# redmod-team/SympGPR

Measured on AMD Instinct MI355X. Metric: Gram-build GB/s + Cholesky fp64 TFLOP/s at N=65536 d=2; |alpha-alpha_ref|/|alpha_ref|, higher is better.
Workload: dtype f64

## Files before the change

include/sympgpr_probe.h:

```cpp
#ifndef SYMPGPR_PROBE_H
#define SYMPGPR_PROBE_H
#include <stddef.h>
#ifdef __cplusplus
extern "C" {
#endif

int sgpr_probe_mfma_f64(int waves_per_simd, int iters, double *tflops);
int sgpr_probe_hbm_write(size_t bytes, int reps, double *gbs);
int sgpr_probe_mfma_clock(int nacc, int waves_per_simd, int iters, double *out3);
int sgpr_probe_gemm(int m, int n, int k, int lower, double *out4);
int sgpr_probe_gemm_debug(int bits);
int sgpr_probe_leaf(double *out8);
int sgpr_probe_lat(double *out8);
int sgpr_probe_xcc(int nblocks, int *host_out);
int sgpr_probe_cumask(const unsigned *mask_words, int nwords, int nblocks, int *host_out);

int sgpr_probe_generated_eval(int family, int which, int m, const double *xa, const double *ya,
                              const double *xb, const double *yb, const double *l, int nl, double *out);

int sgpr_probe_queue_plan(int n, int nworkers, int *starts_out, int max_starts, unsigned *tasks_out, int max_tasks,
                          int *counts);
int sgpr_probe_queue_plan_partial(int n, int nworkers, int nq, int *starts_out, int max_starts, unsigned *tasks_out,
                                  int max_tasks, int *counts);
int sgpr_probe_queue_trace_begin(int max_tasks);
int sgpr_probe_queue_trace_end(unsigned long long *out, int max_tasks);
int sgpr_probe_queue_trace_clear(void);
int sgpr_probe_queue_postmortem(int always);
int sgpr_probe_queue_force_giveup(int on);
int sgpr_probe_tune(const char *name, double value);
int sgpr_probe_strassen_plan(int m, int n, int k, int lower, long smin, long kslab, long scratch_doubles, long long *out,
                             int max_records, int *count);
int sgpr_probe_gemm_strassen_dev(int m, int n, int k, double alpha, const double *A, size_t lda, const double *B, size_t ldb,
                                 double beta, double *C, size_t ldc, int lower, void *stream);
int sgpr_probe_gemm_nt2_dev(int m, int n, int k, double alpha, const double *A, size_t lda, const double *B, size_t ldb,
                            double beta, double *C, size_t ldc, double alpha2, double *C2, size_t ldc2, void *stream);
int sgpr_probe_strassen2_plan(int m, int n, int k, int lower, long smin, long kslab, long smin2, long kslab2, long scratch_doubles,
                              long long *out, int max_records, int *count);
int sgpr_probe_gemm_nt4_dev(int m, int n, int k, const double *A, size_t lda, const double *B, size_t ldb, double beta, int count,
                            double *const *C, const size_t *ldc, const double *alpha, void *stream);
int sgpr_probe_strassen_rec_plan(int m, int n, int k, int lower, long scratch_doubles, long cfg_out[5], long long *out,
                                 int max_records, int *count);
int sgpr_probe_strassen_rec_scratch(int n, unsigned long long out[2]);
int sgpr_probe_gemm_strassen_rec_dev(int m, int n, int k, double alpha, const double *A, size_t lda, const double *B, size_t ldb,
                                     double beta, double *C, size_t ldc, int lower, void *stream);
int sgpr_probe_batch_layout(int path, int mode, int d, int reg, int nbatch, int n_pts, int nhyp, unsigned long long out[24]);
unsigned sgpr_probe_map_calls(void);
int sgpr_probe_map_team(int ntest, int n0);

int sgpr_probe_trsm_piece(int ticket, int cap, int strips, int out[5]);
int sgpr_probe_trsm_counts(int strips, int cap, unsigned long long out[2]);

int sgpr_probe_census(int na, int threads_a, int lds_a, int spin_a, const unsigned *mask_a, int nwords_a,
                      int nb, int threads_b, int lds_b, int spin_b, const unsigned *mask_b, int nwords_b,
                      unsigned long long *host_out);

#ifdef __cplusplus
}
#endif
#endif
```

sympgpr_amd/_lib.py:

```python
import ctypes as C
import os

import numpy as np

FAMILIES = {"A": 0, "B": 1, "C": 2, "D": 3, "USER": 4}
K_KERN, K_DXDX0, K_DYDY0, K_DXDY0 = 0, 1, 2, 3
K_DLX, K_DLY = 4, 8
K_DX, K_DY, K_DX0, K_DY0, K_DXDX0DY0, K_DYDY0DY0, K_DXDY0DY0 = 16, 17, 18, 19, 20, 21, 22
G_QQ, G_PQ, G_QP, G_PP, G_ALL, G_LOWER, G_OCML, G_DLX, G_DLY = 1, 2, 4, 8, 15, 16, 32, 64, 128
FIT_LOWER_ONLY, FIT_REG, FIT_BLOCK_QQ, FIT_BLOCK_PP = 1, 4, 8, 16
MAP_WRAP_Q, MAP_WRAP_P, MAP_EXPLICIT, MAP_LOSS_NEGP = 1, 2, 4, 8
E_ARG, E_NODEVICE, E_HIP, E_NOMEM, E_STATE = -1, -2, -3, -4, -5
LOO_LPD, LOO_PRESS = 0, 1

ABI_VERSION = 5
_dp = C.POINTER(C.c_double)
_vp = C.c_void_p


class SympGPRError(RuntimeError):
    code = None
    detail = ""


# ... 135 lines not shown
    "sgpr_probe_queue_plan_partial": (C.c_int, [C.c_int, C.c_int, C.c_int, C.POINTER(C.c_int), C.c_int, C.POINTER(C.c_uint),
                                                C.c_int, C.POINTER(C.c_int)]),
    "sgpr_probe_queue_trace_begin": (C.c_int, [C.c_int]),
    "sgpr_probe_queue_trace_end": (C.c_int, [C.POINTER(C.c_ulonglong), C.c_int]),
    "sgpr_probe_queue_postmortem": (C.c_int, [C.c_int]),
    "sgpr_probe_queue_force_giveup": (C.c_int, [C.c_int]),
    "sgpr_probe_tune": (C.c_int, [C.c_char_p, C.c_double]),
    "sgpr_probe_map_calls": (C.c_uint, []),
    "sgpr_probe_map_team": (C.c_int, [C.c_int, C.c_int]),
    "sgpr_probe_trsm_piece": (C.c_int, [C.c_int, C.c_int, C.c_int, C.POINTER(C.c_int)]),
    "sgpr_probe_trsm_counts": (C.c_int, [C.c_int, C.c_int, C.POINTER(C.c_ulonglong)]),
    "sgpr_probe_queue_trace_clear": (C.c_int, []),
    "sgpr_probe_strassen_plan": (C.c_int, [C.c_int, C.c_int, C.c_int, C.c_int, C.c_long, C.c_long, C.c_long,
                                           C.POINTER(C.c_longlong), C.c_int, C.POINTER(C.c_int)]),
    "sgpr_probe_gemm_strassen_dev": (C.c_int, [C.c_int, C.c_int, C.c_int, C.c_double, C.c_void_p, C.c_size_t, C.c_void_p, C.c_size_t,
                                               C.c_double, C.c_void_p, C.c_size_t, C.c_int, C.c_void_p]),
    "sgpr_probe_gemm_nt2_dev": (C.c_int, [C.c_int, C.c_int, C.c_int, C.c_double, C.c_void_p, C.c_size_t, C.c_void_p, C.c_size_t,
                                          C.c_double, C.c_void_p, C.c_size_t, C.c_double, C.c_void_p, C.c_size_t, C.c_void_p]),
    "sgpr_probe_strassen2_plan": (C.c_int, [C.c_int, C.c_int, C.c_int, C.c_int, C.c_long, C.c_long, C.c_long, C.c_long, C.c_long,
                                            C.POINTER(C.c_longlong), C.c_int, C.POINTER(C.c_int)]),
    "sgpr_probe_strassen_rec_plan": (C.c_int, [C.c_int, C.c_int, C.c_int, C.c_int, C.c_long, C.POINTER(C.c_long),
                                               C.POINTER(C.c_longlong), C.c_int, C.POINTER(C.c_int)]),
    "sgpr_probe_strassen_rec_scratch": (C.c_int, [C.c_int, C.POINTER(C.c_ulonglong)]),
    "sgpr_probe_gemm_strassen_rec_dev": (C.c_int, [C.c_int, C.c_int, C.c_int, C.c_double, C.c_void_p, C.c_size_t, C.c_void_p, C.c_size_t,
                                                   C.c_double, C.c_void_p, C.c_size_t, C.c_int, C.c_void_p]),
    "sgpr_probe_gemm_nt4_dev": (C.c_int, [C.c_int, C.c_int, C.c_int, C.c_void_p, C.c_size_t, C.c_void_p, C.c_size_t, C.c_double, C.c_int,
                                          C.POINTER(C.c_void_p), C.POINTER(C.c_size_t), C.POINTER(C.c_double), C.c_void_p]),
    "sgpr_probe_batch_layout": (C.c_int, [C.c_int, C.c_int, C.c_int, C.c_int, C.c_int, C.c_int, C.c_int,
                                          C.POINTER(C.c_ulonglong)]),
    "sgpr_probe_census": (C.c_int, [C.c_int, C.c_int, C.c_int, C.c_int, C.POINTER(C.c_uint), C.c_int,
                                    C.c_int, C.c_int, C.c_int, C.c_int, C.POINTER(C.c_uint), C.c_int,
                                    C.POINTER(C.c_ulonglong)]),
}

_LIB = None
_PROBE = None


def load_library():
    global _LIB
    if _LIB is not None:
        return _LIB
    path = lib_path()
    if os.environ.get("SYMPGPR_NO_TORCH_PRELOAD") != "1":
        try:
            import torch
# ... 80 lines not shown
```

sympgpr_amd/csrc/chol.hip:

```cpp
#include <algorithm>
#include <cstdlib>
#include <mutex>
#include <vector>

#include "cholq.h"
#include "common.h"
#include "gemm_tile.h"
#include "leaf.h"

namespace sgpr {

namespace {

using namespace leaf;


__global__ __launch_bounds__(LT) void leaf_kernel(int nb, double *A, size_t lda, double *inv,
                                                  int *dinfo, int goff, int mode,
                                                  unsigned long long *stamps)
{
    __shared__ double s[LEAF_LDS];
    if (nb == LEAF) leaf_body(s, (int)LEAF, A, lda, inv, dinfo, goff, mode, stamps);
    else            leaf_body(s, nb, A, lda, inv, dinfo, goff, mode, stamps);
}
// ... 958 lines not shown
    int dev = -1;
    if (caller) {
        SGPR_HIP(hipStreamGetDevice(caller, &dev));
    } else {
        SGPR_HIP(hipGetDevice(&dev));
    }
    if (dev < 0 || dev >= 64) { set_error("potrf: device index out of range"); return SGPR_E_ARG; }
    std::lock_guard<std::mutex> lock(g_side_mu);
    if (!side[dev]) {
        int cur = -1, lo = 0, hi = 0;
        SGPR_HIP(hipGetDevice(&cur));
        if (cur != dev) SGPR_HIP(hipSetDevice(dev));
        hipError_t e = hipDeviceGetStreamPriorityRange(&lo, &hi);
        if (e == hipSuccess) e = hipStreamCreateWithPriority(&side[dev], hipStreamNonBlocking, hi);
        if (e == hipSuccess) register_exit_release();
        if (cur != dev) (void)hipSetDevice(cur);
        SGPR_HIP(e);
    }
    *out = side[dev];
    *dev_out = dev;
    return 0;
}

struct QueueDevice {
    std::mutex mu;
    hipEvent_t done = nullptr;
    int ncu = 0;
    hipStream_t workers[4] = {}, panels[4] = {};
    bool overlap_ok[4] = {};
    bool failed = false;
};
QueueDevice g_qdev[64];

__global__ void overlap_probe_kernel(int *w, int me)
{
    __hip_atomic_store((gint *)(w + me), 1, __ATOMIC_RELAXED, __HIP_MEMORY_SCOPE_AGENT);
    const unsigned long long t0 = __builtin_amdgcn_s_memrealtime();
    int seen = 0;
    while (!(seen = __hip_atomic_load((gint *)(w + 1 - me), __ATOMIC_RELAXED, __HIP_MEMORY_SCOPE_AGENT))) {
        __builtin_amdgcn_s_sleep(32);
        if (__builtin_amdgcn_s_memrealtime() - t0 > 5000000ull) break;
    }
    w[2 + me] = seen ? 1 : 2;
}
static bool queue_overlap_ok(hipStream_t sw, hipStream_t sp)
{
// ... 117 lines not shown
    cholq::remember(ws, n, (int)(plan->tasks.size() / 2));
    cholq::remember_plan(plan);
    static const bool qdebug = tune("q_debug", 0) != 0;
    if (qdebug) {
        SGPR_HIP(hipStreamSynchronize(su));
        cholq::postmortem(false);
    }
    if (plan->nq < plan->nblk) {
        const int S = plan->starts[plan->nq];
        Ctx ct = c;
        ct.qws = nullptr;
        static const bool nosync = tune("q_nosync", 0) != 0;
        if (!nosync) SGPR_HIP(hipStreamSynchronize(su));
        return potrf_lookahead(n - S, A + S + (size_t)S * lda, lda, ct, 0, off0 + S);
    }
    return 0;
}

void release_all_streams_at_exit()
{
    int ndev = 0;
    if (hipGetDeviceCount(&ndev) != hipSuccess) { (void)hipGetLastError(); return; }
    for (int dev = 0; dev < ndev && dev < 64; ++dev) {
        hipStream_t drop[9] = {};
        int nd = 0;
        {
            std::lock_guard<std::mutex> lock(g_side_mu);
            if (g_side[dev]) { drop[nd++] = g_side[dev]; g_side[dev] = nullptr; }
        }
        {
            QueueDevice &qd = g_qdev[dev];
            std::lock_guard<std::mutex> lock(qd.mu);
            for (int r = 0; r < 4; ++r) {
                if (qd.workers[r]) { drop[nd++] = qd.workers[r]; qd.workers[r] = nullptr; }
                if (qd.panels[r]) { drop[nd++] = qd.panels[r]; qd.panels[r] = nullptr; }
            }
            qd.failed = true;
        }
        if (!nd) continue;
        int cur = -1;
        (void)hipGetDevice(&cur);
        if (cur != dev) (void)hipSetDevice(dev);
        for (int q = 0; q < nd; ++q) (void)hipStreamDestroy(drop[q]);
        if (cur != dev && cur >= 0) (void)hipSetDevice(cur);
    }
    (void)hipGetLastError();
}

int release_streams(int dev)
{
    {
        bool any = false;
        {
            std::lock_guard<std::mutex> lock(g_side_mu);
            any = g_side[dev] != nullptr;
        }
        QueueDevice &qd = g_qdev[dev];
        std::lock_guard<std::mutex> lock(qd.mu);
        for (int r = 0; r < 4; ++r) any = any || qd.workers[r] || qd.panels[r];
        any = any || qd.done;
        if (!any) return 0;
    }
    int cur = -1;
    SGPR_HIP(hipGetDevice(&cur));
    if (cur != dev) SGPR_HIP(hipSetDevice(dev));
    hipError_t first = hipSuccess;
    auto drop = [&](hipStream_t &s) {
        if (!s) return;
        hipError_t e = hipStreamSynchronize(s);
        if (e == hipSuccess) e = hipStreamDestroy(s);
        if (e != hipSuccess && first == hipSuccess) first = e;
        s = nullptr;
    };
    {
        std::lock_guard<std::mutex> lock(g_side_mu);
        drop(g_side[dev]);
    }
    {
        QueueDevice &qd = g_qdev[dev];
        std::lock_guard<std::mutex> lock(qd.mu);
        for (int r = 0; r < 4; ++r) { drop(qd.workers[r]); drop(qd.panels[r]); }
        if (qd.done) {
            const hipError_t e = hipEventDestroy(qd.done);
            if (e != hipSuccess && first == hipSuccess) first = e;
            qd.done = nullptr;
        }
        qd.ncu = 0;
        qd.failed = false;
        for (int r = 0; r < 4; ++r) qd.overlap_ok[r] = false;
    }
    if (cur != dev) (void)hipSetDevice(cur);
    SGPR_HIP(first);
    return 0;
}

int potrf_lookahead(int n, double *A, size_t lda, const Ctx &c, int nb, int off0)
{
    if (nb == 0 && c.qws && c.flags && cholq::eligible(n) && (lda & 1) == 0 && (((uintptr_t)A & 15) == 0) && off0 % LEAF == 0) {
        const int rq = potrf_queue(n, A, lda, c, off0);
// ... 446 lines not shown
```

sympgpr_amd/csrc/common.h:

```cpp
#pragma once
#include <hip/hip_runtime.h>
#include <cstddef>
#include <cstdint>
#include <string>
#include <type_traits>
#include <vector>

#include "../../include/sympgpr_hip.h"

namespace sgpr {

void set_error(const std::string &msg);
double tune(const char *name, double dflt);
void tune_set(const char *name, double v);
int hip_fail(hipError_t e, const char *what, const char *file, int line);

#define SGPR_HIP(call)                                                          \
    do {                                                                        \
        hipError_t e__ = (call);                                                \
        if (e__ != hipSuccess) return ::sgpr::hip_fail(e__, #call, __FILE__, __LINE__); \
    } while (0)

#define SGPR_CHECK_LAUNCH() SGPR_HIP(hipGetLastError())

// ... 84 lines not shown
int gemm_nt_two(int m, int n, int k, double alpha, const double *A, size_t lda, const double *B, size_t ldb, double beta,
             double *C, size_t ldc, double alpha2, double *C2, size_t ldc2, hipStream_t st);
constexpr int STRASSEN_REC = 16;
enum { PLAN_SUM = 1, PLAN_PROD = 2, PLAN_CLASSIC = 3 };
int gemm_nt_strassen(int m, int n, int k, double alpha, const double *A, size_t lda, const double *B, size_t ldb, double beta,
                     double *C, size_t ldc, int lower, hipStream_t st);
int strassen_plan(int m, int n, int k, int lower, long smin, long kslab, size_t scratch_doubles, std::vector<long long> &out);
enum { PLAN2_SUM = 4, PLAN2_PROD = 5 };
int strassen_outer_plan(int m, int n, int k, int lower, long smin, long kslab, long smin2, long kslab2, size_t scratch_doubles,
                   std::vector<long long> &out);
int gemm_nt_multi(int m, int n, int k, const double *A, size_t lda, const double *B, size_t ldb, double beta, int count,
                  double *const *C, const size_t *ldc, const double *alpha, hipStream_t st);
size_t strassen_scratch_doubles(int m, int n, int k, int lower, int levels);
struct StrassenCfg { long smin = -1, kslab = -1, smin2 = -1, kslab2 = -1, smin_under = -1; };
int gemm_nt_strassen_cfg(int m, int n, int k, double alpha, const double *A, size_t lda, const double *B, size_t ldb, double beta,
                         double *C, size_t ldc, int lower, const StrassenCfg &cfg, hipStream_t st);
size_t strassen_scratch_doubles_cfg(int m, int n, int k, int lower, int levels, const StrassenCfg &cfg);
struct StrassenRec { bool on = false; long smin_gemm = 0, smin_syrk = 0, smin2_gemm = 0, smin2_syrk = 0, kslab = 0, kslab2 = 0, kslab2_short = 0; };
StrassenRec strassen_rec_values();
StrassenCfg strassen_rec_cfg(const StrassenRec &v, int k, int lower);
int strassen_rec_plan(int m, int n, int k, int lower, long cfg_out[5], size_t scratch_doubles, std::vector<long long> &out);
int gemm_nt_strassen_rec(int m, int n, int k, double alpha, const double *A, size_t lda, const double *B, size_t ldb, double beta,
                         double *C, size_t ldc, int lower, hipStream_t st);
void potrf_strassen_need(int n, size_t out[2]);
void strassen_reserve(size_t both, size_t one, hipStream_t st);
int strassen_trim();
int gemm_profile_begin();
int gemm_profile_end(double *out12);
int gemm_profile_launches(double *buf, int max_records);
void gemm_set_overlap(int on);
int gemm_nt_diag(int m, int n, int k, double alpha, const double *A, size_t lda, const double *B, size_t ldb,
                 double beta, double *C, size_t ldc, int lower, unsigned long long *stamps, int dbg, hipStream_t st);

constexpr int LEAF = 128;
constexpr int POTRF_HANDOFF_TIMEOUT = -1000001;
constexpr int SOLVE_HANDOFF_TIMEOUT = -1000002;
inline int info_status(int info)
{
    if (info >= 0) return info;
    set_error(info == POTRF_HANDOFF_TIMEOUT ? "potrf: a hand-off inside the panel kernel timed out"
              : info == SOLVE_HANDOFF_TIMEOUT ? "solve: a hand-off between the strips of a triangular solve timed out" : "potrf: internal error");
    return SGPR_E_HIP;
}
size_t potrf_workspace(int n);
int potrf(int n, double *A, size_t lda, void *work, size_t lwork, int *dinfo, hipStream_t st);
size_t potrf_batch_flag_bytes(int nbatch);
// ... 123 lines not shown
```

sympgpr_amd/csrc/gemm_f64.hip:

```cpp
#include <algorithm>
#include <atomic>
#include <cstdlib>
#include <mutex>
#include <type_traits>
#include <vector>

#include "common.h"
#include "gemm_tile.h"

namespace sgpr {

namespace {

struct ProfRec { double flop; int big; int m, n, k, lower, overlap; };
struct Prof {
    std::mutex mu;
    std::atomic<bool> on{false};
    std::vector<hipEvent_t> pool;
    std::vector<ProfRec> recs;
    long dropped = 0;
};
constexpr int PROF_POOL = 8192;
Prof g_prof;
thread_local int t_overlap = 0;
// ... 495 lines not shown
    };
    PlanCfg ci = under_of(c);
    ci.scratch = ~(size_t)0;
    for (size_t i = 0; i + STRASSEN_REC <= plan.size(); i += STRASSEN_REC) {
        const long long *r = &plan[i];
        if (r[0] == PLAN_SUM) sums(r, 0);
        else if (r[0] == PLAN2_SUM) sums(r, 2);
        else if (r[0] == PLAN2_PROD) {
            inner_plan(r, ci, in);
            for (size_t j = 0; j + STRASSEN_REC <= in.size(); j += STRASSEN_REC)
                if (in[j] == PLAN_SUM) sums(&in[j], 0);
        }
    }
    return nd;
}

struct Scratch {
    std::mutex mu;
    double *p = nullptr;
    size_t cap = 0, failed = 0;
    hipEvent_t ev = nullptr;
    hipStream_t last = nullptr;
    bool used = false;
};
Scratch g_scratch[64];

bool scratch_ensure(Scratch &s, size_t need)
{
    static const bool forced_fail = tune("gemm_strassen_noscratch", 0) != 0;
    if (forced_fail) return false;
    if (s.cap >= need) return true;
    if (s.failed && need >= s.failed) return false;
    if (s.p) { (void)hipFree(s.p); s.p = nullptr; s.cap = 0; s.used = false; }
    if (hipMalloc((void **)&s.p, need * sizeof(double)) != hipSuccess) {
        (void)hipGetLastError();
        s.p = nullptr;
        s.failed = need;
        return false;
    }
    s.cap = need;
    return true;
}
int device_of(hipStream_t st)
{
    int dev = -1;
    if ((st ? hipStreamGetDevice(st, &dev) : hipGetDevice(&dev)) != hipSuccess) { (void)hipGetLastError(); return -1; }
    return (dev >= 0 && dev < 64) ? dev : -1;
}

int block_sum(int rows, int cols, const double *X, size_t ldx, const double *Y, size_t ldy, double sign, double *T, hipStream_t st)
{
    const long pieces = (long)((rows + 511) / 512) * ((cols + 3) / 4);
    hipLaunchKernelGGL(block_sum_kernel, dim3((unsigned)std::min(pieces, 2048L)), dim3(256), 0, st, rows, cols, X, ldx, Y, ldy, sign, T);
    SGPR_CHECK_LAUNCH();
    return 0;
}

int run_plan(const long long *recs, size_t nrec, double alpha, const double *A, size_t lda, const double *B, size_t ldb,
             double beta, double *C, size_t ldc, double alpha2, double *C2, size_t ldc2, double *SA, double *SB, hipStream_t st)
{
    for (size_t i = 0; i < nrec; ++i) {
        const long long *r = recs + i * STRASSEN_REC;
        int rc = 0;
        if (r[0] == PLAN_SUM) {
            const double *P = r[1] ? B : A;
            const size_t ld = r[1] ? ldb : lda;
            rc = block_sum((int)r[2], (int)r[3], P + r[4] + (size_t)r[5] * ld, ld, P + r[6] + (size_t)r[7] * ld, ld, (double)r[8],
                           r[1] ? SB : SA, st);
        } else if (r[0] == PLAN_PROD) {
            const int m = (int)r[7], n = (int)r[8], k = (int)r[9];
            const double *Ap = r[1] ? SA : A + r[2] + (size_t)r[3] * lda;
            const double *Bp = r[4] ? SB : B + r[5] + (size_t)r[6] * ldb;
            const size_t la = r[1] ? (size_t)m : lda, lb = r[4] ? (size_t)n : ldb;
            double *C1 = C + r[10] + (size_t)r[11] * ldc;
            if (C2) {
                double *cs[4] = {C1, nullptr, nullptr, nullptr};
                size_t ls[4] = {ldc, 0, 0, 0};
                double as[4] = {alpha * (double)r[12], 0.0, 0.0, 0.0};
                int cnt = 1;
                auto add = [&](double *p, size_t l, double a) { cs[cnt] = p; ls[cnt] = l; as[cnt] = a; ++cnt; };
                if (r[15]) add(C + r[13] + (size_t)r[14] * ldc, ldc, alpha * (double)r[15]);
                add(C2 + r[10] + (size_t)r[11] * ldc2, ldc2, alpha2 * (double)r[12]);
                if (r[15]) add(C2 + r[13] + (size_t)r[14] * ldc2, ldc2, alpha2 * (double)r[15]);
                if (cnt == 2) rc = gemm_nt_two(m, n, k, as[0], Ap, la, Bp, lb, 1.0, cs[0], ls[0], as[1], cs[1], ls[1], st);
                else          rc = gemm_nt_multi(m, n, k, Ap, la, Bp, lb, 1.0, cnt, cs, ls, as, st);
            } else if (r[15]) {
                rc = gemm_nt_two(m, n, k, alpha * (double)r[12], Ap, la, Bp, lb, 1.0, C1, ldc,
                                 alpha * (double)r[15], C + r[13] + (size_t)r[14] * ldc, ldc, st);
            } else {
                rc = gemm_nt(m, n, k, alpha * (double)r[12], Ap, la, Bp, lb, 1.0, C1, ldc, 0, 0, st);
            }
// ... 24 lines not shown
    std::vector<long long> in;
    for (size_t i = 0; i + STRASSEN_REC <= plan.size(); i += STRASSEN_REC) {
        const long long *r = &plan[i];
        int rc = 0;
        if (r[0] == PLAN2_SUM) {
            const double *P = r[1] ? B : A;
            const size_t ld = r[1] ? ldb : lda;
            rc = block_sum((int)r[2], (int)r[3], P + r[4] + (size_t)r[5] * ld, ld, P + r[6] + (size_t)r[7] * ld, ld, (double)r[8],
                           r[1] ? OB : OA, st);
        } else if (r[0] == PLAN2_PROD) {
            const double *X = r[1] ? OA : A + r[2] + (size_t)r[3] * lda;
            const double *Y = r[4] ? OB : B + r[5] + (size_t)r[6] * ldb;
            inner_plan(r, ci, in);
            rc = run_plan(in.data(), in.size() / STRASSEN_REC, alpha * (double)r[12], X, r[1] ? (size_t)r[7] : lda, Y, r[4] ? (size_t)r[8] : ldb,
                          1.0, C + r[10] + (size_t)r[11] * ldc, ldc, alpha * (double)r[15], r[15] ? C + r[13] + (size_t)r[14] * ldc : nullptr, ldc,
                          SA, SB, st);
        } else {
            rc = run_plan(r, 1, alpha, A, lda, B, ldb, beta, C, ldc, 0.0, nullptr, 0, SA, SB, st);
        }
        if (rc) return rc;
    }
    return 0;
}
}

int strassen_plan(int m, int n, int k, int lower, long smin, long kslab, size_t scratch_doubles, std::vector<long long> &out)
{
    if (m < 0 || n < 0 || k < 0 || (lower && m != n)) { set_error("strassen_plan: bad extents"); return SGPR_E_ARG; }
    PlanCfg c = default_cfg();
    if (smin >= 0) c.smin = std::max(128L, smin);
    if (kslab >= 0) c.kslab = std::max(32L, kslab);
    c.scratch = scratch_doubles;
    out.clear();
    if (lower) plan_syrk(n, k, 0, c, out);
    else       plan_gemm(m, n, k, 0, 0, 0, 0, c, out);
    return 0;
}

namespace {
Plan2Cfg cfg2_of(long smin, long kslab, long smin2, long kslab2, size_t scratch_doubles)
{
    Plan2Cfg c = default_cfg2();
    if (smin >= 0) c.in.smin = std::max(128L, smin);
    if (kslab >= 0) c.in.kslab = std::max(32L, kslab);
    if (smin2 >= 0) c.smin2 = std::max(256L, smin2);
    if (kslab2 >= 0) c.kslab2 = std::max(64L, kslab2);
// ... 37 lines not shown
    if (v.kslab2_short < 64 || v.kslab2_short % 64 != 0 || v.kslab2_short >= v.kslab2) v.kslab2_short = 0;
    return v;
}
StrassenCfg strassen_rec_cfg(const StrassenRec &v, int k, int lower)
{
    StrassenCfg c;
    if (!v.on) return c;
    c.smin = lower ? v.smin_syrk : v.smin_gemm;
    c.smin2 = lower ? v.smin2_syrk : v.smin2_gemm;
    c.smin_under = std::min(c.smin, c.smin2 / 2);
    c.kslab = v.kslab;
    c.kslab2 = (k < v.kslab2 && v.kslab2_short > 0 && k >= v.kslab2_short) ? v.kslab2_short : v.kslab2;
    return c;
}
int strassen_rec_plan(int m, int n, int k, int lower, long cfg_out[5], size_t scratch_doubles, std::vector<long long> &out)
{
    if (m < 0 || n < 0 || k < 0 || (lower && m != n)) { set_error("strassen_rec_plan: bad extents"); return SGPR_E_ARG; }
    const Plan2Cfg c = cfg2_of(strassen_rec_cfg(strassen_rec_values(), k, lower), scratch_doubles);
    if (cfg_out) { cfg_out[0] = c.in.smin; cfg_out[1] = c.in.kslab; cfg_out[2] = c.smin2; cfg_out[3] = c.kslab2; cfg_out[4] = under_of(c).smin; }
    outer_plan_of(m, n, k, lower, c, out);
    return 0;
}

size_t strassen_scratch_doubles(int m, int n, int k, int lower, int levels)
{
    return strassen_scratch_doubles_cfg(m, n, k, lower, levels, StrassenCfg{});
}
size_t strassen_scratch_doubles_cfg(int m, int n, int k, int lower, int levels, const StrassenCfg &cfg)
{
    std::vector<long long> plan;
    if (!strassen_on() || m < 0 || n < 0 || k < 0 || (lower && m != n)) return 0;
    const Plan2Cfg c2 = cfg2_of(cfg, ~(size_t)0);
    if (levels >= 2 && strassen_levels() >= 2) {
        outer_plan_of(m, n, k, lower, c2, plan);
        return plan2_need(plan, c2).total();
    }
    if (strassen_plan(m, n, k, lower, c2.in.smin, c2.in.kslab, ~(size_t)0, plan)) return 0;
    return plan_need(plan);
}

void strassen_reserve(size_t both, size_t one, hipStream_t st)
{
    const int dev = device_of(st);
    if (dev < 0 || !strassen_on()) return;
    Scratch &s = g_scratch[dev];
    std::lock_guard<std::mutex> lock(s.mu);
    if (both > one && !outer_noscratch() && scratch_ensure(s, both)) return;
    if (one) (void)scratch_ensure(s, one);
}

int strassen_trim()
{
    for (Scratch &s : g_scratch) {
        std::lock_guard<std::mutex> lock(s.mu);
        if (s.p) (void)hipFree(s.p);
        if (s.ev) (void)hipEventDestroy(s.ev);
        s.p = nullptr; s.ev = nullptr; s.cap = 0; s.failed = 0; s.used = false; s.last = nullptr;
    }
    (void)hipGetLastError();
    return 0;
}

int gemm_nt_strassen(int m, int n, int k, double alpha, const double *A, size_t lda, const double *B, size_t ldb, double beta,
                     double *C, size_t ldc, int lower, hipStream_t st)
{
    return gemm_nt_strassen_cfg(m, n, k, alpha, A, lda, B, ldb, beta, C, ldc, lower, StrassenCfg{}, st);
}
int gemm_nt_strassen_rec(int m, int n, int k, double alpha, const double *A, size_t lda, const double *B, size_t ldb, double beta,
                         double *C, size_t ldc, int lower, hipStream_t st)
{
    return gemm_nt_strassen_cfg(m, n, k, alpha, A, lda, B, ldb, beta, C, ldc, lower, strassen_rec_cfg(strassen_rec_values(), k, lower), st);
}
int gemm_nt_strassen_cfg(int m, int n, int k, double alpha, const double *A, size_t lda, const double *B, size_t ldb, double beta,
                         double *C, size_t ldc, int lower, const StrassenCfg &cfg, hipStream_t st)
{
    const Plan2Cfg c2 = cfg2_of(cfg, ~(size_t)0);
    const bool aligned = ((((uintptr_t)A | (uintptr_t)B) & 15) == 0) && (((lda | ldb) & 1) == 0);
    if (std::min(m, n) / 2 < std::min(c2.in.smin, under_of(c2).smin) || !strassen_on() || !aligned || beta != 1.0 || (lower && m != n))
        return gemm_nt(m, n, k, alpha, A, lda, B, ldb, beta, C, ldc, lower, 0, st);
    std::vector<long long> plan;
    int rc = 0;
    const int dev = device_of(st);
    auto enqueue = [&](Scratch &s, auto &&run) {
        if (!s.ev) SGPR_HIP(hipEventCreateWithFlags(&s.ev, hipEventDisableTiming));
        if (s.used && s.last != st) SGPR_HIP(hipStreamWaitEvent(st, s.ev, 0));
        const int r = run();
        SGPR_HIP(hipEventRecord(s.ev, st));
        s.last = st;
        s.used = true;
        return r;
    };
    if (strassen_levels() >= 2 && dev >= 0 && !outer_noscratch() && std::min(lower ? m / 2 : m, lower ? n / 2 : n) / 2 >= c2.smin2) {
        outer_plan_of(m, n, k, lower, c2, plan);
        const Need2 nd = plan2_need(plan, c2);
        if (nd.v[2] + nd.v[3]) {
            Scratch &s = g_scratch[dev];
            std::lock_guard<std::mutex> lock(s.mu);
            if (scratch_ensure(s, nd.total()))
                return enqueue(s, [&] { return run_plan2(plan, c2, nd, alpha, A, lda, B, ldb, beta, C, ldc, s.p, st); });
        }
    }
    rc = strassen_plan(m, n, k, lower, c2.in.smin, c2.in.kslab, ~(size_t)0, plan);
    if (rc) return rc;
    const size_t need = plan_need(plan);
    if (!need) return run_plan(plan, alpha, A, lda, B, ldb, beta, C, ldc, nullptr, nullptr, st);
    if (dev < 0) return gemm_nt(m, n, k, alpha, A, lda, B, ldb, beta, C, ldc, lower, 0, st);
    Scratch &s = g_scratch[dev];
    std::lock_guard<std::mutex> lock(s.mu);
    if (!scratch_ensure(s, need)) {
        if ((rc = strassen_plan(m, n, k, lower, c2.in.smin, c2.in.kslab, s.cap, plan))) return rc;
        if (!plan_need(plan)) return run_plan(plan, alpha, A, lda, B, ldb, beta, C, ldc, nullptr, nullptr, st);
    }
    size_t na = 0;
    for (size_t i = 0; i + STRASSEN_REC <= plan.size(); i += STRASSEN_REC)
        if (plan[i] == PLAN_SUM && plan[i + 1] == 0) na = std::max(na, (size_t)plan[i + 2] * (size_t)plan[i + 3]);
    return enqueue(s, [&] { return run_plan(plan, alpha, A, lda, B, ldb, beta, C, ldc, s.p, s.p + na, st); });
}

}
```

sympgpr_amd/csrc/probe.hip:

```cpp
#include <algorithm>
#include <cstdlib>
#include <vector>

#include "cholq.h"
#include "common.h"
#include "../../include/sympgpr_probe.h"
#include "generated/pair_generated.h"
#include "nd_eval.h"

namespace sgpr {
namespace {
typedef double double4_t __attribute__((ext_vector_type(4)));
typedef double double2_t __attribute__((ext_vector_type(2)));

template <int NACC>
__global__ __launch_bounds__(256) void mfma_clock_kernel(int iters, double *out, unsigned long long *stamps)
{
    double4_t acc[NACC];
    const double a = 1.0 + threadIdx.x * 1e-9, b = 1.0 - threadIdx.x * 1e-9;
#pragma unroll
    for (int i = 0; i < NACC; ++i) acc[i] = double4_t{0.0, 0.0, 0.0, 0.0};
    const unsigned long long t0 = __builtin_amdgcn_s_memtime(), r0 = __builtin_amdgcn_s_memrealtime();
    for (int it = 0; it < iters; ++it) {
#pragma unroll
// ... 508 lines not shown
    *count = (int)(plan.size() / STRASSEN_REC);
    for (size_t i = 0; out && i < plan.size() && (int)(i / STRASSEN_REC) < max_records; ++i) out[i] = plan[i];
    return 0;
}
extern "C" int sgpr_probe_strassen_rec_plan(int m, int n, int k, int lower, long scratch_doubles, long cfg_out[5], long long *out,
                                            int max_records, int *count)
{
    if (!count || scratch_doubles < 0) { set_error("probe_strassen_rec_plan: bad arguments"); return SGPR_E_ARG; }
    std::vector<long long> plan;
    const int rc = strassen_rec_plan(m, n, k, lower, cfg_out, (size_t)scratch_doubles, plan);
    if (rc) return rc;
    *count = (int)(plan.size() / STRASSEN_REC);
    for (size_t i = 0; out && i < plan.size() && (int)(i / STRASSEN_REC) < max_records; ++i) out[i] = plan[i];
    return 0;
}
extern "C" int sgpr_probe_strassen_rec_scratch(int n, unsigned long long out[2])
{
    if (n < 0 || !out) { set_error("probe_strassen_rec_scratch: bad arguments"); return SGPR_E_ARG; }
    size_t need[2];
    potrf_strassen_need(n, need);
    out[0] = need[0]; out[1] = need[1];
    return 0;
}
extern "C" int sgpr_probe_gemm_strassen_rec_dev(int m, int n, int k, double alpha, const double *A, size_t lda, const double *B, size_t ldb,
                                                double beta, double *C, size_t ldc, int lower, void *stream)
{
    return gemm_nt_strassen_rec(m, n, k, alpha, A, lda, B, ldb, beta, C, ldc, lower, static_cast<hipStream_t>(stream));
}
extern "C" int sgpr_probe_gemm_nt4_dev(int m, int n, int k, const double *A, size_t lda, const double *B, size_t ldb, double beta,
                                       int count, double *const *C, const size_t *ldc, const double *alpha, void *stream)
{
    return gemm_nt_multi(m, n, k, A, lda, B, ldb, beta, count, C, ldc, alpha, static_cast<hipStream_t>(stream));
}
extern "C" int sgpr_probe_batch_layout(int path, int mode, int d, int reg, int nbatch, int n_pts, int nhyp, unsigned long long out[24])
{
    const long n = d ? 2L * d * n_pts : reg ? (long)n_pts : 2L * n_pts;
    if (path < 0 || path > 1 || mode < 0 || mode > 3 || (path && mode == 3) || d < 0 || d > 3 || (d && (reg || mode)) || nbatch < 1 ||
        n_pts < 1 || nhyp < 1 || (path ? n <= 256 || n > 2048 : n > 256) || !out) {
        set_error("probe_batch_layout: bad arguments");
        return SGPR_E_ARG;
    }
    const BatchLayout l = batch_layout(path, mode, d, reg, nbatch, n_pts, nhyp);
    const size_t v[24] = {(size_t)l.chunk, l.nacc, l.o_x, l.o_y, l.o_z, l.o_kc, l.o_no, l.in_bytes, l.o_al, l.o_nll, l.o_info, l.out_bytes,
                          l.o_A, l.o_inv, l.o_fl, l.o_fl2, l.o_r, l.o_pub, l.o_st, l.o_part, l.scr_bytes,
                          sizeof(KConst), sizeof(nd::NdConst), l.flag_bytes};
    for (int i = 0; i < 24; ++i) out[i] = v[i];
// ... 61 lines not shown
```

Measured before the change: 80.77.

## Overlap Strassen block sums with products on side streams via scheduled dependencies

Adds a scheduler that turns the Strassen GEMM plan into records carrying explicit buffer dependencies. Block-sum kernels run on low-priority side streams with a reduced workgroup count, synchronised through pooled events, so they overlap with the MFMA product kernels on the main stream. When spare scratch exists, each scratch region gets two buffers so the next sum can fill one while a product still reads the other. The overlap is on by default and adds event and stream-wait overhead plus the risk that side-stream sums compete with the GEMMs for compute units.

```diff
diff --git a/include/sympgpr_probe.h b/include/sympgpr_probe.h
--- a/include/sympgpr_probe.h
+++ b/include/sympgpr_probe.h
@@ -43,6 +43,8 @@
 int sgpr_probe_strassen_rec_scratch(int n, unsigned long long out[2]);
 int sgpr_probe_gemm_strassen_rec_dev(int m, int n, int k, double alpha, const double *A, size_t lda, const double *B, size_t ldb,
                                      double beta, double *C, size_t ldc, int lower, void *stream);
+int sgpr_probe_strassen_schedule(int m, int n, int k, int lower, long capacity_doubles, long long info[12], long long *out,
+                                 int max_records, int *count);
 int sgpr_probe_batch_layout(int path, int mode, int d, int reg, int nbatch, int n_pts, int nhyp, unsigned long long out[24]);
 unsigned sgpr_probe_map_calls(void);
 int sgpr_probe_map_team(int ntest, int n0);
diff --git a/sympgpr_amd/_lib.py b/sympgpr_amd/_lib.py
--- a/sympgpr_amd/_lib.py
+++ b/sympgpr_amd/_lib.py
@@ -181,6 +181,8 @@
     "sgpr_probe_strassen_rec_plan": (C.c_int, [C.c_int, C.c_int, C.c_int, C.c_int, C.c_long, C.POINTER(C.c_long),
                                                C.POINTER(C.c_longlong), C.c_int, C.POINTER(C.c_int)]),
     "sgpr_probe_strassen_rec_scratch": (C.c_int, [C.c_int, C.POINTER(C.c_ulonglong)]),
+    "sgpr_probe_strassen_schedule": (C.c_int, [C.c_int, C.c_int, C.c_int, C.c_int, C.c_long, C.POINTER(C.c_longlong),
+                                               C.POINTER(C.c_longlong), C.c_int, C.POINTER(C.c_int)]),
     "sgpr_probe_gemm_strassen_rec_dev": (C.c_int, [C.c_int, C.c_int, C.c_int, C.c_double, C.c_void_p, C.c_size_t, C.c_void_p, C.c_size_t,
                                                    C.c_double, C.c_void_p, C.c_size_t, C.c_int, C.c_void_p]),
     "sgpr_probe_gemm_nt4_dev": (C.c_int, [C.c_int, C.c_int, C.c_int, C.c_void_p, C.c_size_t, C.c_void_p, C.c_size_t, C.c_double, C.c_int,
diff --git a/sympgpr_amd/csrc/chol.hip b/sympgpr_amd/csrc/chol.hip
--- a/sympgpr_amd/csrc/chol.hip
+++ b/sympgpr_amd/csrc/chol.hip
@@ -1004,6 +1004,37 @@
     return 0;
 }
 
+hipStream_t g_sum[64][2] = {};
+}
+
+int strassen_sum_streams(hipStream_t caller, int count, hipStream_t *out)
+{
+    int dev = -1;
+    if (caller) {
+        SGPR_HIP(hipStreamGetDevice(caller, &dev));
+    } else {
+        SGPR_HIP(hipGetDevice(&dev));
+    }
+    if (dev < 0 || dev >= 64 || count < 1 || count > 2) { set_error("strassen_sum_streams: bad device or count"); return SGPR_E_ARG; }
+    std::lock_guard<std::mutex> lock(g_side_mu);
+    for (int t = 0; t < count; ++t) {
+        if (!g_sum[dev][t]) {
+            int cur = -1, lo = 0, hi = 0;
+            SGPR_HIP(hipGetDevice(&cur));
+            if (cur != dev) SGPR_HIP(hipSetDevice(dev));
+            hipError_t e = hipDeviceGetStreamPriorityRange(&lo, &hi);
+            if (e == hipSuccess) e = hipStreamCreateWithPriority(&g_sum[dev][t], hipStreamNonBlocking, lo);
+            if (e == hipSuccess) register_exit_release();
+            if (cur != dev) (void)hipSetDevice(cur);
+            SGPR_HIP(e);
+        }
+        out[t] = g_sum[dev][t];
+    }
+    return 0;
+}
+
+namespace {
+
 struct QueueDevice {
     std::mutex mu;
     hipEvent_t done = nullptr;
@@ -1167,11 +1198,12 @@
     int ndev = 0;
     if (hipGetDeviceCount(&ndev) != hipSuccess) { (void)hipGetLastError(); return; }
     for (int dev = 0; dev < ndev && dev < 64; ++dev) {
-        hipStream_t drop[9] = {};
+        hipStream_t drop[11] = {};
         int nd = 0;
         {
             std::lock_guard<std::mutex> lock(g_side_mu);
             if (g_side[dev]) { drop[nd++] = g_side[dev]; g_side[dev] = nullptr; }
+            for (hipStream_t &s : g_sum[dev]) if (s) { drop[nd++] = s; s = nullptr; }
         }
         {
             QueueDevice &qd = g_qdev[dev];
@@ -1198,7 +1230,7 @@
         bool any = false;
         {
             std::lock_guard<std::mutex> lock(g_side_mu);
-            any = g_side[dev] != nullptr;
+            any = g_side[dev] != nullptr || g_sum[dev][0] != nullptr || g_sum[dev][1] != nullptr;
         }
         QueueDevice &qd = g_qdev[dev];
         std::lock_guard<std::mutex> lock(qd.mu);
@@ -1220,6 +1252,8 @@
     {
         std::lock_guard<std::mutex> lock(g_side_mu);
         drop(g_side[dev]);
+        drop(g_sum[dev][0]);
+        drop(g_sum[dev][1]);
     }
     {
         QueueDevice &qd = g_qdev[dev];
diff --git a/sympgpr_amd/csrc/common.h b/sympgpr_amd/csrc/common.h
--- a/sympgpr_amd/csrc/common.h
+++ b/sympgpr_amd/csrc/common.h
@@ -130,6 +130,9 @@
 int strassen_rec_plan(int m, int n, int k, int lower, long cfg_out[5], size_t scratch_doubles, std::vector<long long> &out);
 int gemm_nt_strassen_rec(int m, int n, int k, double alpha, const double *A, size_t lda, const double *B, size_t ldb, double beta,
                          double *C, size_t ldc, int lower, hipStream_t st);
+constexpr int SCHED_REC = 32;
+int strassen_schedule(int m, int n, int k, int lower, long long cap_doubles, long long info[12], std::vector<long long> &out);
+int strassen_sum_streams(hipStream_t caller, int count, hipStream_t *out);
 void potrf_strassen_need(int n, size_t out[2]);
 void strassen_reserve(size_t both, size_t one, hipStream_t st);
 int strassen_trim();
diff --git a/sympgpr_amd/csrc/gemm_f64.hip b/sympgpr_amd/csrc/gemm_f64.hip
--- a/sympgpr_amd/csrc/gemm_f64.hip
+++ b/sympgpr_amd/csrc/gemm_f64.hip
@@ -541,6 +541,7 @@
     hipEvent_t ev = nullptr;
     hipStream_t last = nullptr;
     bool used = false;
+    std::vector<hipEvent_t> pool;
 };
 Scratch g_scratch[64];
 
@@ -567,16 +568,19 @@
     return (dev >= 0 && dev < 64) ? dev : -1;
 }
 
-int block_sum(int rows, int cols, const double *X, size_t ldx, const double *Y, size_t ldy, double sign, double *T, hipStream_t st)
+constexpr long SUM_WGS = 2048;
+int block_sum(int rows, int cols, const double *X, size_t ldx, const double *Y, size_t ldy, double sign, double *T, hipStream_t st,
+              long wgs = SUM_WGS)
 {
     const long pieces = (long)((rows + 511) / 512) * ((cols + 3) / 4);
-    hipLaunchKernelGGL(block_sum_kernel, dim3((unsigned)std::min(pieces, 2048L)), dim3(256), 0, st, rows, cols, X, ldx, Y, ldy, sign, T);
+    hipLaunchKernelGGL(block_sum_kernel, dim3((unsigned)std::min(pieces, wgs)), dim3(256), 0, st, rows, cols, X, ldx, Y, ldy, sign, T);
     SGPR_CHECK_LAUNCH();
     return 0;
 }
 
 int run_plan(const long long *recs, size_t nrec, double alpha, const double *A, size_t lda, const double *B, size_t ldb,
-             double beta, double *C, size_t ldc, double alpha2, double *C2, size_t ldc2, double *SA, double *SB, hipStream_t st)
+             double beta, double *C, size_t ldc, double alpha2, double *C2, size_t ldc2, double *SA, double *SB, hipStream_t st,
+             long sum_wgs = SUM_WGS)
 {
     for (size_t i = 0; i < nrec; ++i) {
         const long long *r = recs + i * STRASSEN_REC;
@@ -585,7 +589,7 @@
             const double *P = r[1] ? B : A;
             const size_t ld = r[1] ? ldb : lda;
             rc = block_sum((int)r[2], (int)r[3], P + r[4] + (size_t)r[5] * ld, ld, P + r[6] + (size_t)r[7] * ld, ld, (double)r[8],
-                           r[1] ? SB : SA, st);
+                           r[1] ? SB : SA, st, sum_wgs);
         } else if (r[0] == PLAN_PROD) {
             const int m = (int)r[7], n = (int)r[8], k = (int)r[9];
             const double *Ap = r[1] ? SA : A + r[2] + (size_t)r[3] * lda;
@@ -656,6 +660,174 @@
     }
     return 0;
 }
+
+struct SchedCfg {
+    int nbuf[4] = {1, 1, 1, 1};
+    size_t off[4][2] = {};
+    int nstreams = 1;
+};
+SchedCfg sched_cfg_of(const Need2 &nd, size_t cap)
+{
+    SchedCfg sc;
+    sc.nstreams = tune("gemm_strassen_overlap_streams", 1) >= 2 ? 2 : 1;
+    const double lim = tune("gemm_strassen_overlap_slack", -1);
+    size_t slack = cap > nd.total() ? cap - nd.total() : 0, pos = 0;
+    if (lim >= 0) slack = std::min(slack, (size_t)lim);
+    for (int r = 0; r < 4; ++r) { sc.off[r][0] = pos; pos += nd.v[r]; }
+    for (int r = 0; r < 4; ++r) {
+        if (!nd.v[r]) continue;
+        if (nd.v[r] > slack) break;
+        sc.nbuf[r] = 2; sc.off[r][1] = pos; pos += nd.v[r]; slack -= nd.v[r];
+    }
+    return sc;
+}
+void schedule_of(const std::vector<long long> &plan, const Plan2Cfg &c, const Need2 &nd, const SchedCfg &sc, std::vector<long long> &out)
+{
+    struct Buf { long long writer = -1, prod_reader = -1, sum_reader[2] = {-1, -1}; };
+    Buf buf[4][2];
+    int next[4] = {0, 0, 0, 0}, cur[4] = {0, 0, 0, 0};
+    out.clear();
+    auto emit = [&](const long long *r, int level) {
+        const size_t at = out.size();
+        out.resize(at + SCHED_REC, 0);
+        for (int j = 0; j < STRASSEN_REC; ++j) out[at + j] = r[j];
+        out[at + 16] = level; out[at + 18] = out[at + 19] = -1;
+        return at;
+    };
+    auto wait = [&](size_t at, long long idx) {
+        if (idx < 0) return;
+        const int nw = (int)out[at + 20];
+        for (int j = 0; j < nw; ++j) if (out[at + 21 + j] == idx) return;
+        if (nw < SCHED_REC - 21) { out[at + 21 + nw] = idx; out[at + 20] = nw + 1; }
+    };
+    auto read = [&](size_t at, int rg, int b) {
+        wait(at, buf[rg][b].writer);
+        buf[rg][b].prod_reader = (long long)(at / SCHED_REC);
+    };
+    auto sum = [&](const long long *r, int level, int rg, int src, int sb) {
+        const size_t at = emit(r, level);
+        const long long idx = (long long)(at / SCHED_REC);
+        const int stream = sc.nstreams == 2 ? 1 + (int)r[1] : 1, b = next[rg];
+        next[rg] = (b + 1) % sc.nbuf[rg];
+        Buf &t = buf[rg][b];
+        wait(at, t.prod_reader); wait(at, t.sum_reader[0]); wait(at, t.sum_reader[1]);
+        if (!out[at + 20]) wait(at, t.writer);
+        if (src >= 0) { wait(at, buf[src][sb].writer); buf[src][sb].sum_reader[stream - 1] = idx; }
+        t = Buf{};
+        t.writer = idx;
+        cur[rg] = b;
+        out[at + 17] = stream; out[at + 18] = b;
+    };
+    PlanCfg ci = under_of(c);
+    ci.scratch = nd.inner();
+    std::vector<long long> in;
+    for (size_t i = 0; i + STRASSEN_REC <= plan.size(); i += STRASSEN_REC) {
+        const long long *r = &plan[i];
+        if (r[0] == PLAN_SUM || r[0] == PLAN2_SUM) {
+            sum(r, 0, (r[0] == PLAN2_SUM ? 2 : 0) + (int)r[1], -1, 0);
+        } else if (r[0] == PLAN_PROD) {
+            const size_t at = emit(r, 0);
+            if (r[1]) { out[at + 18] = cur[0]; read(at, 0, cur[0]); }
+            if (r[4]) { out[at + 19] = cur[1]; read(at, 1, cur[1]); }
+        } else if (r[0] == PLAN2_PROD) {
+            const size_t hd = emit(r, 0);
+            const int xa = r[1] ? cur[2] : -1, yb = r[4] ? cur[3] : -1;
+            out[hd + 18] = xa; out[hd + 19] = yb;
+            inner_plan(r, ci, in);
+            for (size_t j = 0; j + STRASSEN_REC <= in.size(); j += STRASSEN_REC) {
+                const long long *q = &in[j];
+                if (q[0] == PLAN_SUM) {
+                    const int ob = q[1] ? yb : xa;
+                    sum(q, 1, (int)q[1], ob >= 0 ? 2 + (int)q[1] : -1, std::max(ob, 0));
+                    continue;
+                }
+                const size_t at = emit(q, 1);
+                const bool a_scr = q[0] == PLAN_PROD && q[1], b_scr = q[0] == PLAN_PROD && q[4];
+                if (a_scr) { out[at + 18] = cur[0]; read(at, 0, cur[0]); } else if (xa >= 0) read(at, 2, xa);
+                if (b_scr) { out[at + 19] = cur[1]; read(at, 1, cur[1]); } else if (yb >= 0) read(at, 3, yb);
+            }
+        } else {
+            (void)emit(r, 0);
+        }
+    }
+}
+
+bool overlap_on() { return tune("gemm_strassen_overlap", 1) != 0; }
+constexpr long SUM_WGS_SIDE = 256;
+
+int run_schedule(const std::vector<long long> &plan, const Plan2Cfg &c, const Need2 &nd, double alpha, const double *A, size_t lda,
+                 const double *B, size_t ldb, double beta, double *C, size_t ldc, Scratch &s, hipStream_t st)
+{
+    const SchedCfg sc = sched_cfg_of(nd, s.cap);
+    std::vector<long long> sch;
+    schedule_of(plan, c, nd, sc, sch);
+    const size_t nrec = sch.size() / SCHED_REC;
+    const long wgs = std::min(65535L, std::max(1L, (long)tune("gemm_strassen_sum_wgs", (double)SUM_WGS_SIDE)));
+    hipStream_t str[3] = {st, nullptr, nullptr};
+    int rc = strassen_sum_streams(st, sc.nstreams, str + 1);
+    if (rc) return rc;
+    std::vector<char> needs(nrec, 0);
+    for (size_t i = 0; i < nrec; ++i) {
+        const long long *q = &sch[i * SCHED_REC];
+        for (int j = 0; j < (int)q[20]; ++j)
+            if (sch[(size_t)q[21 + j] * SCHED_REC + 17] != q[17]) needs[(size_t)q[21 + j]] = 1;
+    }
+    if (s.pool.size() < nrec + 2) s.pool.resize(nrec + 2, nullptr);
+    auto event = [&](size_t i) {
+        if (!s.pool[i]) SGPR_HIP(hipEventCreateWithFlags(&s.pool[i], hipEventDisableTiming));
+        return 0;
+    };
+    if ((rc = event(0)) || (rc = event(1))) return rc;
+    SGPR_HIP(hipEventRecord(s.pool[0], st));
+    for (int t = 1; t <= sc.nstreams; ++t) SGPR_HIP(hipStreamWaitEvent(str[t], s.pool[0], 0));
+    struct Join {
+        hipStream_t *str; int n; hipEvent_t *ev;
+        ~Join()
+        {
+            for (int t = 1; t <= n; ++t)
+                if (hipEventRecord(ev[t - 1], str[t]) != hipSuccess || hipStreamWaitEvent(str[0], ev[t - 1], 0) != hipSuccess) {
+                    (void)hipGetLastError();
+                    (void)hipStreamSynchronize(str[t]);
+                }
+        }
+    } join{str, sc.nstreams, s.pool.data()};
+    auto at = [&](int rg, long long b) { return s.p + sc.off[rg][b < 0 ? 0 : b]; };
+    const long long *hd = nullptr;
+    for (size_t i = 0; i < nrec; ++i) {
+        const long long *q = &sch[i * SCHED_REC];
+        hipStream_t me = str[q[17]];
+        for (int j = 0; j < (int)q[20]; ++j) {
+            const size_t w = (size_t)q[21 + j];
+            if (sch[w * SCHED_REC + 17] != q[17]) SGPR_HIP(hipStreamWaitEvent(me, s.pool[2 + w], 0));
+        }
+        if (q[0] == PLAN2_PROD) {
+            hd = q;
+            continue;
+        }
+        if (q[0] == PLAN2_SUM) {
+            const double *P = q[1] ? B : A;
+            const size_t ld = q[1] ? ldb : lda;
+            rc = block_sum((int)q[2], (int)q[3], P + q[4] + (size_t)q[5] * ld, ld, P + q[6] + (size_t)q[7] * ld, ld, (double)q[8],
+                           at(2 + (int)q[1], q[18]), me, wgs);
+        } else if (q[16] == 0) {
+            rc = run_plan(q, 1, alpha, A, lda, B, ldb, beta, C, ldc, 0.0, nullptr, 0, at(0, q[0] == PLAN_SUM && q[1] ? 0 : q[18]),
+                          at(1, q[0] == PLAN_SUM ? q[18] : q[19]), me, wgs);
+        } else {
+            const long long *r = hd;
+            const double *X = r[1] ? at(2, r[18]) : A + r[2] + (size_t)r[3] * lda;
+            const double *Y = r[4] ? at(3, r[19]) : B + r[5] + (size_t)r[6] * ldb;
+            rc = run_plan(q, 1, alpha * (double)r[12], X, r[1] ? (size_t)r[7] : lda, Y, r[4] ? (size_t)r[8] : ldb, 1.0,
+                          C + r[10] + (size_t)r[11] * ldc, ldc, alpha * (double)r[15], r[15] ? C + r[13] + (size_t)r[14] * ldc : nullptr, ldc,
+                          at(0, q[0] == PLAN_SUM && q[1] ? 0 : q[18]), at(1, q[0] == PLAN_SUM ? q[18] : q[19]), me, wgs);
+        }
+        if (rc) return rc;
+        if (needs[i]) {
+            if ((rc = event(2 + i))) return rc;
+            SGPR_HIP(hipEventRecord(s.pool[2 + i], me));
+        }
+    }
+    return 0;
+}
 }
 
 int strassen_plan(int m, int n, int k, int lower, long smin, long kslab, size_t scratch_doubles, std::vector<long long> &out)
@@ -739,6 +911,29 @@
     return 0;
 }
 
+int strassen_schedule(int m, int n, int k, int lower, long long cap_doubles, long long info[12], std::vector<long long> &out)
+{
+    if (m < 0 || n < 0 || k < 0 || (lower && m != n)) { set_error("strassen_schedule: bad extents"); return SGPR_E_ARG; }
+    const Plan2Cfg c = cfg2_of(strassen_rec_cfg(strassen_rec_values(), k, lower), ~(size_t)0);
+    std::vector<long long> plan;
+    if (strassen_levels() >= 2 && !outer_noscratch()) outer_plan_of(m, n, k, lower, c, plan);
+    else {
+        const int rc = strassen_plan(m, n, k, lower, c.in.smin, c.in.kslab, ~(size_t)0, plan);
+        if (rc) return rc;
+    }
+    const Need2 nd = plan2_need(plan, c);
+    const size_t cap = cap_doubles < 0 ? nd.total() : (size_t)cap_doubles;
+    if (cap < nd.total()) { set_error("strassen_schedule: the capacity is below the call's need"); return SGPR_E_ARG; }
+    const SchedCfg sc = sched_cfg_of(nd, cap);
+    schedule_of(plan, c, nd, sc, out);
+    if (info) {
+        for (int i = 0; i < 12; ++i) info[i] = 0;
+        for (int r = 0; r < 4; ++r) { info[r] = (long long)nd.v[r]; info[4 + r] = sc.nbuf[r]; }
+        info[8] = sc.nstreams; info[9] = (long long)cap;
+    }
+    return 0;
+}
+
 size_t strassen_scratch_doubles(int m, int n, int k, int lower, int levels)
 {
     return strassen_scratch_doubles_cfg(m, n, k, lower, levels, StrassenCfg{});
@@ -772,6 +967,8 @@
         std::lock_guard<std::mutex> lock(s.mu);
         if (s.p) (void)hipFree(s.p);
         if (s.ev) (void)hipEventDestroy(s.ev);
+        for (hipEvent_t e : s.pool) if (e) (void)hipEventDestroy(e);
+        s.pool.clear();
         s.p = nullptr; s.ev = nullptr; s.cap = 0; s.failed = 0; s.used = false; s.last = nullptr;
     }
     (void)hipGetLastError();
@@ -798,6 +995,7 @@
     std::vector<long long> plan;
     int rc = 0;
     const int dev = device_of(st);
+    const bool overlap = overlap_on();
     auto enqueue = [&](Scratch &s, auto &&run) {
         if (!s.ev) SGPR_HIP(hipEventCreateWithFlags(&s.ev, hipEventDisableTiming));
         if (s.used && s.last != st) SGPR_HIP(hipStreamWaitEvent(st, s.ev, 0));
@@ -814,7 +1012,10 @@
             Scratch &s = g_scratch[dev];
             std::lock_guard<std::mutex> lock(s.mu);
             if (scratch_ensure(s, nd.total()))
-                return enqueue(s, [&] { return run_plan2(plan, c2, nd, alpha, A, lda, B, ldb, beta, C, ldc, s.p, st); });
+                return enqueue(s, [&] {
+                    return overlap ? run_schedule(plan, c2, nd, alpha, A, lda, B, ldb, beta, C, ldc, s, st)
+                                   : run_plan2(plan, c2, nd, alpha, A, lda, B, ldb, beta, C, ldc, s.p, st);
+                });
         }
     }
     rc = strassen_plan(m, n, k, lower, c2.in.smin, c2.in.kslab, ~(size_t)0, plan);
@@ -828,10 +1029,9 @@
         if ((rc = strassen_plan(m, n, k, lower, c2.in.smin, c2.in.kslab, s.cap, plan))) return rc;
         if (!plan_need(plan)) return run_plan(plan, alpha, A, lda, B, ldb, beta, C, ldc, nullptr, nullptr, st);
     }
-    size_t na = 0;
-    for (size_t i = 0; i + STRASSEN_REC <= plan.size(); i += STRASSEN_REC)
-        if (plan[i] == PLAN_SUM && plan[i + 1] == 0) na = std::max(na, (size_t)plan[i + 2] * (size_t)plan[i + 3]);
-    return enqueue(s, [&] { return run_plan(plan, alpha, A, lda, B, ldb, beta, C, ldc, s.p, s.p + na, st); });
-}
-
-}
+    const Need2 nd = plan2_need(plan, c2);
+    if (overlap) return enqueue(s, [&] { return run_schedule(plan, c2, nd, alpha, A, lda, B, ldb, beta, C, ldc, s, st); });
+    return enqueue(s, [&] { return run_plan(plan, alpha, A, lda, B, ldb, beta, C, ldc, s.p, s.p + nd.v[0], st); });
+}
+
+}
diff --git a/sympgpr_amd/csrc/probe.hip b/sympgpr_amd/csrc/probe.hip
--- a/sympgpr_amd/csrc/probe.hip
+++ b/sympgpr_amd/csrc/probe.hip
@@ -554,6 +554,17 @@
     out[0] = need[0]; out[1] = need[1];
     return 0;
 }
+extern "C" int sgpr_probe_strassen_schedule(int m, int n, int k, int lower, long capacity_doubles, long long info[12], long long *out,
+                                            int max_records, int *count)
+{
+    if (!count) { set_error("probe_strassen_schedule: bad arguments"); return SGPR_E_ARG; }
+    std::vector<long long> sched;
+    const int rc = strassen_schedule(m, n, k, lower, (long long)capacity_doubles, info, sched);
+    if (rc) return rc;
+    *count = (int)(sched.size() / SCHED_REC);
+    for (size_t i = 0; out && i < sched.size() && (int)(i / SCHED_REC) < max_records; ++i) out[i] = sched[i];
+    return 0;
+}
 extern "C" int sgpr_probe_gemm_strassen_rec_dev(int m, int n, int k, double alpha, const double *A, size_t lda, const double *B, size_t ldb,
                                                 double beta, double *C, size_t ldc, int lower, void *stream)
 {
```

New measurement: 82.37, median of 6. 1.02x the previous value.
